# erikszasz/GaussianSplattingRegistration

Hardware: AMD Instinct MI355X
Metric: Gaussians/sec through HEM level + ICP iters/sec, 2x5M-splat pair (higher is better)
Workload: dtype f32 (HEM) / f64 (ICP)

## Files before the change

### gaussiansplattingregistration_amd/csrc/icp.hip

```cpp
#include "gsr_common.h"
#include "gsr_normals.h"
#include "gsr_solve.h"
#include "gsr_features.h"
#include "gsr_grid.h"
#include "gsr_oneshot.h"
#include "gsr_prims.h"

#include <float.h>
#include <math.h>
#include <stdlib.h>
#include <string.h>
#include <vector>

namespace gsr {
#ifndef GSR_ICP_MERGE_BS
#define GSR_ICP_MERGE_BS 1024
#define GSR_ICP_MERGE_IPT 4
#endif
using icp_merge_cfg = rocprim::merge_sort_config<512, GSR_ICP_MERGE_BS, GSR_ICP_MERGE_IPT, 128, 128, 4>;
using icp_sort_cfg = rocprim::radix_sort_config<rocprim::default_config, icp_merge_cfg,
                                                rocprim::radix_sort_onesweep_config<rocprim::kernel_config<1024, 16>, rocprim::kernel_config<1024, 16>, 11,
                                                                                    rocprim::block_radix_rank_algorithm::match>>;

#ifndef ICP_CELL_FLOOR_DIV
// ... 951 lines not shown
    const bool first = s_st.evals == 0;
    const bool stop = !first && fabs(s_st.fit - fit) < s_st.rel_fit && fabs(s_st.rmse - rmse) < s_st.rel_rmse;
    st->fit = fit; st->rmse = rmse;
    st->evals = s_st.evals + 1;
    if (stop || s_st.iters >= s_st.max_iter) { st->done = 1; return; }
    double update[16], T[16];
    estimate_update(s_st.ctr, s_st.kind, acc, update);
#pragma unroll
    for (int i = 0; i < 16; ++i) T[i] = s_st.T[i];
    mat4_mul(update, T, T);
#pragma unroll
    for (int i = 0; i < 16; ++i) st->T[i] = T[i];
    st->iters = s_st.iters + 1;
}
__global__ __launch_bounds__(ICP_STEP_THREADS) void k_icp_step(int nblocks, const double* __restrict__ partials, const double* __restrict__ reduced,
                                                   IcpState* __restrict__ st) {
    __shared__ double s_x[16][GSR_ICP_ACC_LEN];
    __shared__ IcpState s_st;
    static_assert(GSR_ICP_ACC_LEN == 32 && sizeof(IcpState) % 4 == 0, "k_icp_step layout");
    if (threadIdx.x < sizeof(IcpState) / 4) reinterpret_cast<int*>(&s_st)[threadIdx.x] = reinterpret_cast<const int*>(st)[threadIdx.x];
    icp_fold_partials<ICP_STEP_THREADS>(nblocks, partials, reduced, s_x);
    if (threadIdx.x != 0 || s_st.done) return;
    icp_step_solve(&s_x[0][0], s_st, st);
}

__global__ __launch_bounds__(1024) void k_icp_reduce(int nblocks, const double* __restrict__ partials, const IcpState* __restrict__ st,
                                                     double* __restrict__ out) {
    const int lane = threadIdx.x & 63, wv = threadIdx.x >> 6;
    const bool done = st->done != 0;
    for (int k = wv; k < GSR_ICP_ACC_LEN; k += 16) {
        double s = 0.0;
        if (!done)
            for (int b = lane; b < nblocks; b += 64) s += partials[(int64_t)b * GSR_ICP_ACC_LEN + k];
        for (int o = 32; o > 0; o >>= 1) s += __shfl_xor(s, o);
        if (lane == 0) out[k] = s;
    }
}

// ... 3 lines not shown

struct gsr_icp_ctx {
    int device = 0;
    hipStream_t stream = nullptr;
    IcpGrid grid;
    bool have_target = false, have_normals = false, have_source = false;
    int64_t nt = 0, ns = 0, ns_global = 0;
    double max_corr = 0;
    DevBuf src_raw, src_order, state, nn_j, Tc, Sc, stage_cov, Ti, Tg, Si;
    bool have_tcov = false, have_scov = false, have_tcol = false, have_scol = false;
    double lambda_geometric = 0.968;
    bool src_sorted = false;
    bool device_loop = true;
    bool block_search = true;
    bool xcd_ranges = true;
    gsr_comm* comm = nullptr;
    PinnedBlock host_rb;
    unsigned long long rb_seq = 0;
    int nn_kernel = -1;
    int nn_mode() const { return nn_kernel >= 0 ? (nn_kernel ? 2 : 0) : (ns >= 400000 ? 2 : 0); }
    double cell_target = 2.0;
    DevBuf hist;
    bool robust_box = false;
    bool robust_allowed = true;
    DevBuf bbox, keys, idx, skeys, order, cellStart, Tq, Tn, stage_xyz, stage_nrm, src, partials, acc_dev, rocprim_tmp, corr_idx, corr_d2;
    gsr_allreduce_fn allreduce = nullptr;
    void* allreduce_user = nullptr;
    gsr_allreduce_dev64_fn allreduce_dev = nullptr;
    void* allreduce_dev_user = nullptr;
    Event e0, e1, eb0, eb1;
    bool defer_sync = false;
    bool build_pending = false;
    float ms_build = 0, ms_iter = 0;
// ... 51 lines not shown
    const double* tn = p2p ? nullptr : (kind == GSR_ICP_GENERALIZED ? c->Tc.as<double>() : c->Tn.as<double>());
    const double* sc = kind == GSR_ICP_GENERALIZED ? c->Sc.as<double>() : nullptr;
    decltype(&k_icp_accumulate_dev<0, 0>) kernel = nullptr;
    switch (2 * kind + (blockf ? 1 : 0)) {
        case 0: kernel = k_icp_accumulate_dev<0, 0>; break;
        case 1: kernel = k_icp_accumulate_dev<0, 1>; break;
        case 2: kernel = k_icp_accumulate_dev<1, 0>; break;
        case 3: kernel = k_icp_accumulate_dev<1, 1>; break;
        case 4: kernel = k_icp_accumulate_dev<2, 0>; break;
        case 5: kernel = k_icp_accumulate_dev<2, 1>; break;
        case 6: kernel = k_icp_accumulate_dev<3, 0>; break;
        case 7: kernel = k_icp_accumulate_dev<3, 1>; break;
        case 8: kernel = k_icp_accumulate_dev<4, 0>; break;
        default: kernel = k_icp_accumulate_dev<4, 1>; break;
    }
    hipLaunchKernelGGL(kernel, dim3(8 * ((nb + 7) / 8)), dim3(256), 0, st, c->ns, c->src.as<float>(), c->state.as<IcpState>(), c->grid, c->cellStart.as<int>(), nnj,
                       c->Tq.as<float4>(), tn, sc, cargs, mc2, loss, k, c->partials.as<double>(), c->xcd_ranges ? nb : -nb);
}

int32_t run_accumulate(gsr_icp_ctx* c, const double* T, int kind, int loss, double k, double* acc, bool timed) {
    GSR_TRY(icp_check_kind(c, kind));
    hipStream_t st = c->stream;
    Xform X;
    for (int i = 0; i < 12; ++i) X.m[i] = T[i];
    const int nb = icp_blocks(c->ns, c->nblocks);
    GSR_TRY(c->partials.reserve((size_t)nb * GSR_ICP_ACC_LEN * 8));
    GSR_TRY(c->acc_dev.reserve(GSR_ICP_ACC_LEN * 8));
    GSR_HIP(hipMemsetAsync(c->partials.p, 0, (size_t)nb * GSR_ICP_ACC_LEN * 8, st));
    if (timed) GSR_HIP(hipEventRecord(c->e0, st));
    const double mc2 = c->max_corr * c->max_corr;
    const int* nnj = nullptr;
// ... 51 lines not shown
    unsigned* const host_rb = c->host_rb.as<unsigned>();
    if (!host_rb || bytes > 1024 || (bytes & 3)) {
        GSR_HIP(hipMemcpyAsync(out, dev, bytes, hipMemcpyDeviceToHost, st));
        GSR_HIP(hipStreamSynchronize(st));
        return GSR_OK;
    }
    const unsigned long long seq = ++c->rb_seq;
    unsigned long long* flag = reinterpret_cast<unsigned long long*>(host_rb + 256);
    hipLaunchKernelGGL(k_icp_publish, dim3(1), dim3(64), 0, st, (const unsigned*)dev, (int)(bytes >> 2), host_rb, flag, seq);
    GSR_HIP(hipGetLastError());
    GSR_TRY(wait_host_flag(st, flag, seq, true));
    memcpy(out, (const void*)host_rb, bytes);
    return GSR_OK;
}

int32_t gsr_icp_create(gsr_icp_ctx** out, int32_t device, void* stream) {
    if (!out) return fail(GSR_E_INVALID, "gsr_icp_create: out is NULL");
    *out = nullptr;
    int ndev = 0;
    if (hipGetDeviceCount(&ndev) != hipSuccess || ndev <= 0)
        return fail(GSR_E_NO_DEVICE, "gsr_icp_create: no HIP device visible (this backend has no CPU fallback)");
    if (device < 0 || device >= ndev) return fail(GSR_E_INVALID, "gsr_icp_create: device %d out of range", device);
    GSR_HIP(hipSetDevice(device));
    gsr_icp_ctx* c = new gsr_icp_ctx();
    c->device = device;
    c->stream = (hipStream_t)stream;
    if (c->e0.create() != hipSuccess || c->e1.create() != hipSuccess || c->eb0.create() != hipSuccess || c->eb1.create() != hipSuccess) {
        delete c; return fail(GSR_E_HIP, "hipEventCreate failed");
    }
    if (const char* e = getenv("GSR_ICP_DEVICE_LOOP")) c->device_loop = atoi(e) != 0;
    if (const char* e = getenv("GSR_ICP_BLOCK_SEARCH")) c->block_search = atoi(e) != 0;
    if (const char* e = getenv("GSR_ICP_XCD")) c->xcd_ranges = atoi(e) != 0;
    if (const char* e = getenv("GSR_ICP_ROBUST_BOX")) c->robust_allowed = atoi(e) != 0;
    if (const char* e = getenv("GSR_ICP_BLOCKS")) { int v = atoi(e); if (v >= 1 && v <= 65536) c->nblocks = v; }
    bool poll = true;
    if (const char* e = getenv("GSR_ICP_RB_POLL")) poll = atoi(e) != 0;
    if (!poll || c->host_rb.alloc(1024 + 64) != hipSuccess) (void)hipGetLastError();
    if (const char* e = getenv("GSR_ICP_NN_KERNEL")) c->nn_kernel = atoi(e);
    if (const char* e = getenv("GSR_ICP_CELL_TARGET")) { double v = atof(e); if (v > 0.01 && v < 1000) c->cell_target = v; }
    if (const char* e = getenv("GSR_ICP_MAX_CELLS")) { int v = atoi(e); if (v >= 1024) c->max_cells = v; }
    *out = c;
    return GSR_OK;
}

int32_t gsr_icp_destroy(gsr_icp_ctx* c) {
    delete c;
    return GSR_OK;
}

int32_t gsr_icp_set_target(gsr_icp_ctx* c, const float* xyz, const double* normals, int64_t n, double max_corr, int32_t on_device) {
    if (!c) return fail(GSR_E_INVALID, "gsr_icp_set_target: NULL context");
    if (!(max_corr > 0)) return fail(GSR_E_PRECONDITION, "max_correspondence_distance must be > 0 (got %g)", max_corr);
    if (n <= 0 || !xyz) return fail(GSR_E_PRECONDITION, "gsr_icp_set_target: empty target cloud");
    if (n >= ((int64_t)1 << 31) - 1) return fail(GSR_E_INVALID, "gsr_icp_set_target: n too large");
    GSR_HIP(hipSetDevice(c->device));
    hipStream_t st = c->stream;
    GSR_HIP(hipEventRecord(c->eb0, st));
    const float* dxyz = xyz;
    const double* dnrm = normals;
    if (!on_device) {
        GSR_TRY(c->stage_xyz.reserve((size_t)n * 12));
        GSR_HIP(hipMemcpyAsync(c->stage_xyz.p, xyz, (size_t)n * 12, hipMemcpyHostToDevice, st));
        dxyz = c->stage_xyz.as<float>();
        if (normals) {
            GSR_TRY(c->stage_nrm.reserve((size_t)n * 24));
            GSR_HIP(hipMemcpyAsync(c->stage_nrm.p, normals, (size_t)n * 24, hipMemcpyHostToDevice, st));
            dnrm = c->stage_nrm.as<double>();
        }
    }
    const int nbb = stride_grid(n);
    GSR_TRY(c->bbox.reserve(64 + (size_t)nbb * 24));
    hipLaunchKernelGGL(k_icp_bbox, dim3(nbb), dim3(256), 0, st, n, dxyz, c->bbox.as<float>() + 16);
    hipLaunchKernelGGL(k_icp_bbox_reduce, dim3(1), dim3(256), 0, st, nbb, c->bbox.as<float>() + 16, c->bbox.as<float>());
    GSR_TRY(c->hist.reserve(3 * ICP_HIST_BINS * 4));
    GSR_HIP(hipMemsetAsync(c->hist.p, 0, 3 * ICP_HIST_BINS * 4, st));
    hipLaunchKernelGGL(k_icp_hist, dim3(nbb > 512 ? 512 : nbb), dim3(256), 0, st, n, dxyz, c->bbox.as<float>(), c->hist.as<unsigned>());
    hipLaunchKernelGGL(k_icp_trim, dim3(1), dim3(64), 0, st, c->hist.as<unsigned>(), c->bbox.as<float>(), c->bbox.as<float>() + 6, c->bbox.as<float>() + 12);
    float hb[13];
    GSR_TRY(icp_fetch(c, c->bbox.p, hb, 13 * 4));
    const float raw_box[6] = {hb[0], hb[1], hb[2], hb[3], hb[4], hb[5]};
    c->robust_box = hb[12] != 0.0f && c->robust_allowed;
    if (c->robust_box) {
        GSR_HIP(hipMemsetAsync(c->hist.p, 0, 3 * ICP_HIST_BINS * 4, st));
        hipLaunchKernelGGL(k_icp_hist, dim3(nbb > 512 ? 512 : nbb), dim3(256), 0, st, n, dxyz, c->bbox.as<float>() + 6, c->hist.as<unsigned>());
        hipLaunchKernelGGL(k_icp_trim, dim3(1), dim3(64), 0, st, c->hist.as<unsigned>(), c->bbox.as<float>() + 6, c->bbox.as<float>(), c->bbox.as<float>() + 12);
        GSR_TRY(icp_fetch(c, c->bbox.p, hb, 6 * 4));
    }
    double mn[3], mx[3];
    for (int k = 0; k < 3; ++k) { mn[k] = hb[k]; mx[k] = hb[3 + k]; }
    IcpGrid g;
    if (!(mx[0] >= mn[0])) { mn[0] = mn[1] = mn[2] = 0; mx[0] = mx[1] = mx[2] = 0; }
    double cell;
    {
        const double ex = mx[0] - mn[0], ey = mx[1] - mn[1], ez = mx[2] - mn[2];
        const double emax = fmax(ex, fmax(ey, ez)), eps = emax * 1e-6 + 1e-30;
        cell = cbrt((ex + eps) * (ey + eps) * (ez + eps) * c->cell_target / (double)n);
        if (!(cell > 0)) cell = max_corr;
        if (cell < max_corr / ICP_CELL_FLOOR_DIV) cell = max_corr / ICP_CELL_FLOOR_DIV;
    }
    GSR_TRY(c->keys.reserve(n * 4)); GSR_TRY(c->idx.reserve(n * 4)); GSR_TRY(c->skeys.reserve(n * 4)); GSR_TRY(c->order.reserve(n * 4));
    for (;;) {
        double fx = floor((mx[0] - mn[0]) / cell) + 1, fy = floor((mx[1] - mn[1]) / cell) + 1, fz = floor((mx[2] - mn[2]) / cell) + 1;
        if (fx * fy * fz <= (double)c->max_cells) { g.gx = (int)fx; g.gy = (int)fy; g.gz = (int)fz; break; }
        cell *= 1.2599210498948732;
    }
    g.ox = mn[0]; g.oy = mn[1]; g.oz = mn[2];
    g.c = cell; g.inv_c = 1.0 / cell;
    g.cx = 0.5 * (mn[0] + mx[0]); g.cy = 0.5 * (mn[1] + mx[1]); g.cz = 0.5 * (mn[2] + mx[2]);
    g.ncells = g.gx * g.gy * g.gz;
    g.rings = (int)ceil(max_corr / cell);
    if (g.rings < 1) g.rings = 1;
    g.bx0 = raw_box[0]; g.by0 = raw_box[1]; g.bz0 = raw_box[2]; g.bx1 = raw_box[3]; g.by1 = raw_box[4]; g.bz1 = raw_box[5];
    if (!(raw_box[3] >= raw_box[0])) { g.bx0 = g.by0 = g.bz0 = -1.0 / 0.0; g.bx1 = g.by1 = g.bz1 = 1.0 / 0.0; }
    hipLaunchKernelGGL(k_icp_keys, dim3(stride_grid(n)), dim3(256), 0, st, n, dxyz, g, c->keys.as<unsigned>(), c->idx.as<unsigned>());
    int bits = 1;
    while (bits < 32 && ((int64_t)1 << bits) < g.ncells) ++bits;
    GSR_TRY(sort_pairs_by_key<icp_sort_cfg>(c->rocprim_tmp, st, c->keys.as<unsigned>(), c->skeys.as<unsigned>(), c->idx.as<unsigned>(),
                                            c->order.as<unsigned>(), (size_t)n, 0u, (unsigned)bits));
    GSR_TRY(c->cellStart.reserve(((size_t)g.ncells + 1) * 4));
    hipLaunchKernelGGL(k_icp_cell_starts, dim3(stride_grid(n)), dim3(256), 0, st, n, c->skeys.as<unsigned>(), (int64_t)g.ncells, c->cellStart.as<int>());
    c->grid = g;
    GSR_TRY(c->Tq.reserve((size_t)n * 16));
    if (normals) GSR_TRY(c->Tn.reserve((size_t)n * 24));
    hipLaunchKernelGGL(k_icp_gather_target, dim3(stride_grid(n)), dim3(256), 0, st, n, c->order.as<unsigned>(), dxyz, dnrm,
                       c->Tq.as<float4>(), normals ? c->Tn.as<double>() : (double*)nullptr);
    GSR_HIP(hipEventRecord(c->eb1, st));
    if (c->defer_sync) c->build_pending = true;
    else {
        GSR_HIP(hipStreamSynchronize(st));
        (void)hipEventElapsedTime(&c->ms_build, c->eb0, c->eb1);
        c->build_pending = false;
    }
    GSR_HIP(hipGetLastError());
    c->nt = n; c->max_corr = max_corr; c->have_target = true; c->have_normals = normals != nullptr;
    c->have_tcov = false; c->have_scov = false; c->have_tcol = false; c->have_scol = false;
    c->have_source = false;
    return GSR_OK;
}

int32_t gsr_icp_set_source(gsr_icp_ctx* c, const float* xyz, int64_t n, int32_t on_device) {
    if (!c) return fail(GSR_E_INVALID, "gsr_icp_set_source: NULL context");
    if (n < 0 || (n > 0 && !xyz)) return fail(GSR_E_PRECONDITION, "gsr_icp_set_source: empty source cloud");
    if (n >= ((int64_t)1 << 31) - 1) return fail(GSR_E_INVALID, "gsr_icp_set_source: n too large");
    GSR_HIP(hipSetDevice(c->device));
    hipStream_t st = c->stream;
    GSR_TRY(c->src.reserve((size_t)(n > 0 ? n : 1) * 12));
    c->src_sorted = false;
    if (n == 0) {
    } else if (c->have_target) {
        const float* raw = xyz;
        if (!on_device) {
            GSR_TRY(c->src_raw.reserve((size_t)n * 12));
            GSR_HIP(hipMemcpyAsync(c->src_raw.p, xyz, (size_t)n * 12, hipMemcpyHostToDevice, st));
            raw = c->src_raw.as<float>();
        }
        GSR_TRY(c->keys.reserve(n * 4)); GSR_TRY(c->idx.reserve(n * 4)); GSR_TRY(c->skeys.reserve(n * 4)); GSR_TRY(c->src_order.reserve(n * 4));
        hipLaunchKernelGGL(k_icp_keys, dim3(stride_grid(n)), dim3(256), 0, st, n, raw, c->grid, c->keys.as<unsigned>(), c->idx.as<unsigned>());
        int bits = 1;
// ... 116 lines not shown
    return GSR_OK;
}
int32_t gsr_icp_set_allreduce(gsr_icp_ctx* c, gsr_allreduce_fn fn, void* user, int64_t n_source_global) {
    if (!c) return fail(GSR_E_INVALID, "gsr_icp_set_allreduce: NULL context");
    c->allreduce = fn; c->allreduce_user = user;
    if (fn) { c->allreduce_dev = nullptr; c->allreduce_dev_user = nullptr; c->comm = nullptr; }
    c->ns_global = fn ? n_source_global : c->ns;
    return GSR_OK;
}

int32_t gsr_icp_accumulate(gsr_icp_ctx* c, const double* T, int32_t kind, int32_t loss, double k, double* acc) {
    GSR_TRY(icp_check_scaled(kind, loss, "gsr_icp_accumulate"));
    if (!c || !T || !acc) return fail(GSR_E_INVALID, "gsr_icp_accumulate: NULL argument");
    GSR_HIP(hipSetDevice(c->device));
    return run_accumulate(c, T, kind, loss, k, acc, false);
}

int32_t gsr_icp_register(gsr_icp_ctx* c, const double* init_T, int32_t kind, int32_t loss, double k, double rel_fitness,
                         double rel_rmse, int32_t max_iter, double* out_T, double* fitness, double* inlier_rmse, int32_t* iterations) {
    GSR_TRY(icp_check_scaled(kind, loss, "gsr_icp_register"));
    if (!c || !init_T || !out_T) return fail(GSR_E_INVALID, "gsr_icp_register: NULL argument");
    GSR_HIP(hipSetDevice(c->device));
    c->ms_iter = 0; c->n_iter_kernels = 0;
    const bool multi = c->allreduce_dev != nullptr || c->comm != nullptr;
    if (!c->allreduce && !multi && c->have_source && c->ns == 0)
        return fail(GSR_E_PRECONDITION, "gsr_icp_register: empty source cloud");
    if (!c->allreduce && (c->device_loop || multi)) {
        GSR_TRY(icp_check_kind(c, kind));
        hipStream_t st = c->stream;
        IcpState hs;
        memset(&hs, 0, sizeof(hs));
        memcpy(hs.T, init_T, sizeof(hs.T));
        hs.ctr[0] = c->grid.cx; hs.ctr[1] = c->grid.cy; hs.ctr[2] = c->grid.cz;
        hs.nsg = (double)(multi ? c->ns_global : c->ns); hs.rel_fit = rel_fitness; hs.rel_rmse = rel_rmse;
        hs.max_iter = max_iter < 0 ? 0 : max_iter; hs.kind = kind;
        GSR_TRY(c->state.reserve(sizeof(IcpState)));
        GSR_HIP(hipMemcpyAsync(c->state.p, &hs, sizeof(hs), hipMemcpyHostToDevice, st));
        const int nb = icp_blocks(c->ns, c->nblocks);
        GSR_TRY(c->partials.reserve((size_t)nb * GSR_ICP_ACC_LEN * 8));
        GSR_TRY(c->nn_j.reserve((size_t)(c->ns > 0 ? c->ns : 1) * 4));
        GSR_TRY(c->acc_dev.reserve(GSR_ICP_ACC_LEN * 8));
        GSR_HIP(hipMemsetAsync(c->partials.p, 0, (size_t)nb * GSR_ICP_ACC_LEN * 8, st));
        const double mc2 = c->max_corr * c->max_corr;
        const ColorArgs cargs = {c->Ti.as<double>(), c->Tg.as<double>(), c->Si.as<double>(), sqrt(c->lambda_geometric), sqrt(1.0 - c->lambda_geometric)};
        const int total_evals = hs.max_iter + 1;
        const bool blockf = c->block_search && c->grid.rings >= 2;
        int issued = 0;
        GSR_HIP(hipEventRecord(c->e0, st));
        while (issued < total_evals) {
            const int chunk = total_evals - issued < 8 ? total_evals - issued : 8;
            const int* nnj = c->nn_mode() ? c->nn_j.as<int>() : (const int*)nullptr;
            for (int i = 0; i < chunk; ++i) {
                if (c->nn_mode()) launch_icp_nn<true>(c, st, Xform(), c->state.as<IcpState>(), mc2, blockf);
                launch_accumulate_dev(c, st, kind, blockf, nb, nnj, cargs, mc2, loss, k);
                if (multi) {
                    hipLaunchKernelGGL(k_icp_reduce, dim3(1), dim3(1024), 0, st, nb, c->partials.as<double>(), c->state.as<IcpState>(), c->acc_dev.as<double>());
                    if (c->comm) {
                        GSR_TRY(gsr_comm_allreduce(c->comm, c->acc_dev.p, GSR_ICP_ACC_LEN, GSR_DT_F64, GSR_OP_SUM, (void*)st));
                    } else {
                        const int32_t rc = c->allreduce_dev(c->acc_dev.p, GSR_ICP_ACC_LEN, c->allreduce_dev_user);
                        if (rc != 0) return fail(GSR_E_INVALID, "icp: device all-reduce callback returned %d", rc);
                    }
                    hipLaunchKernelGGL(k_icp_step, dim3(1), dim3(ICP_STEP_THREADS), 0, st, nb, c->partials.as<double>(), c->acc_dev.as<double>(), c->state.as<IcpState>());
                } else {
                    hipLaunchKernelGGL(k_icp_step, dim3(1), dim3(ICP_STEP_THREADS), 0, st, nb, c->partials.as<double>(), (const double*)nullptr, c->state.as<IcpState>());
                }
            }
            issued += chunk;
            GSR_HIP(hipGetLastError());
            GSR_TRY(icp_fetch(c, c->state.p, &hs, sizeof(hs)));
            if (hs.done) break;
        }
        GSR_HIP(hipEventRecord(c->e1, st));
        GSR_HIP(hipStreamSynchronize(st));
        (void)hipEventElapsedTime(&c->ms_iter, c->e0, c->e1);
        c->n_iter_kernels = hs.evals;
        memcpy(out_T, hs.T, sizeof(hs.T));
        if (fitness) *fitness = hs.fit;
        if (inlier_rmse) *inlier_rmse = hs.rmse;
        if (iterations) *iterations = hs.iters;
        return GSR_OK;
    }
    double T[16], acc[GSR_ICP_ACC_LEN], update[16];
    memcpy(T, init_T, sizeof(T));
    GSR_TRY(run_accumulate(c, T, kind, loss, k, acc, true));
    const double nsg = (double)(c->ns_global > 0 ? c->ns_global : c->ns);
    double fit = acc[0] > 0 ? acc[0] / nsg : 0.0, rmse = acc[0] > 0 ? sqrt(acc[1] / acc[0]) : 0.0;
// ... 106 lines not shown
    if (!c) return fail(GSR_E_INVALID, "gsr_icp_register_clouds: NULL context");
    if (kind != GSR_ICP_POINT_TO_POINT && kind != GSR_ICP_POINT_TO_PLANE && kind != GSR_ICP_POINT_TO_POINT_SCALED)
        return fail(GSR_E_INVALID, "gsr_icp_register_clouds: point-to-point and point-to-plane only (covariances / colours: the step-by-step entry points)");
    if (kind == GSR_ICP_POINT_TO_PLANE && !tgt_normals) return fail(GSR_E_PRECONDITION, "TransformationEstimationPointToPlane requires target normals");
    c->comm = nullptr; c->allreduce = nullptr; c->allreduce_user = nullptr; c->allreduce_dev = nullptr; c->allreduce_dev_user = nullptr;
    c->defer_sync = c->device_loop;
    int32_t r = gsr_icp_set_target(c, tgt_xyz, kind == GSR_ICP_POINT_TO_PLANE ? tgt_normals : nullptr, nt, max_corr, on_device);
    if (r == GSR_OK) r = gsr_icp_set_source(c, src_xyz, ns, on_device);
    c->defer_sync = false;
    if (r == GSR_OK) { c->ns_global = ns; r = gsr_icp_register(c, init_T, kind, loss, k, rel_fitness, rel_rmse, max_iter, out_T, fitness, inlier_rmse, iterations); }
    if (r != GSR_OK) (void)hipStreamSynchronize(c->stream);
    icp_read_build_ms(c);
    return r;
}

int32_t gsr_icp_register_multiscale(gsr_icp_ctx* c, int32_t n_entries, const gsr_icp_entry* entries, int32_t on_device, const double* init_T, int32_t kind,
                                    int32_t loss, double k, double rel_fitness, double rel_rmse, gsr_icp_entry_result* results, double* out_T) {
    GSR_TRY(icp_check_scaled(kind, loss, "gsr_icp_register_multiscale"));
    if (!c || !init_T || !out_T || n_entries < 0 || (n_entries > 0 && (!entries || !results)))
        return fail(GSR_E_INVALID, "gsr_icp_register_multiscale: bad argument");
    double T[16];
    memcpy(T, init_T, sizeof(T));
    for (int e = 0; e < n_entries; ++e) {
        const gsr_icp_entry& E = entries[e];
        gsr_icp_entry_result& R = results[e];
        memset(&R, 0, sizeof(R));
        memcpy(R.init_T, T, sizeof(T));
        const int32_t r = gsr_icp_register_clouds(c, E.src_xyz, E.ns, E.tgt_xyz, E.tgt_normals, E.nt, on_device, E.max_corr, T, kind, loss, k, rel_fitness, rel_rmse,
                                                  E.max_iter, R.T, &R.fitness, &R.inlier_rmse, &R.iterations);
        if (r != GSR_OK) return r;
        R.ms_build = c->ms_build; R.ms_iters = c->ms_iter; R.evaluations = c->n_iter_kernels;
        memcpy(T, R.T, sizeof(T));
    }
    memcpy(out_T, T, sizeof(T));
    return GSR_OK;
// ... 159 lines not shown
```

Baseline: 577.0 million.

## Pipeline multiscale ICP levels on device with per-level state slots and host-word polling

Multiscale registration now computes every level's target bounding box in one batch, then enqueues each level's index build, source upload and device ICP loop back to back on the stream. Each level keeps its own state slot, and the next level's starting transform is chained on device from the previous slot, so the host does not synchronise between levels. A state-init kernel replaces the host-to-device state copy and the partials memset. The step kernel also writes a sequence-and-done word to host memory for cheaper polling. This removes host round-trips and stalls between levels, at the cost of more complex control flow and buffers sized to the largest level.

```diff
diff --git a/gaussiansplattingregistration_amd/csrc/icp.hip b/gaussiansplattingregistration_amd/csrc/icp.hip
--- a/gaussiansplattingregistration_amd/csrc/icp.hip
+++ b/gaussiansplattingregistration_amd/csrc/icp.hip
@@ -7,6 +7,7 @@
 #include "gsr_prims.h"
 
 #include <float.h>
+#include <stddef.h>
 #include <math.h>
 #include <stdlib.h>
 #include <string.h>
@@ -989,14 +990,15 @@
     st->iters = s_st.iters + 1;
 }
 __global__ __launch_bounds__(ICP_STEP_THREADS) void k_icp_step(int nblocks, const double* __restrict__ partials, const double* __restrict__ reduced,
-                                                   IcpState* __restrict__ st) {
+                                                   IcpState* __restrict__ st, unsigned long long* __restrict__ host_word, unsigned long long eval_seq) {
     __shared__ double s_x[16][GSR_ICP_ACC_LEN];
     __shared__ IcpState s_st;
     static_assert(GSR_ICP_ACC_LEN == 32 && sizeof(IcpState) % 4 == 0, "k_icp_step layout");
     if (threadIdx.x < sizeof(IcpState) / 4) reinterpret_cast<int*>(&s_st)[threadIdx.x] = reinterpret_cast<const int*>(st)[threadIdx.x];
     icp_fold_partials<ICP_STEP_THREADS>(nblocks, partials, reduced, s_x);
-    if (threadIdx.x != 0 || s_st.done) return;
-    icp_step_solve(&s_x[0][0], s_st, st);
+    if (threadIdx.x != 0) return;
+    if (!s_st.done) icp_step_solve(&s_x[0][0], s_st, st);
+    if (host_word) __hip_atomic_store(host_word, 2ull * eval_seq + (st->done != 0 ? 1ull : 0ull), __ATOMIC_RELAXED, __HIP_MEMORY_SCOPE_SYSTEM);
 }
 
 __global__ __launch_bounds__(1024) void k_icp_reduce(int nblocks, const double* __restrict__ partials, const IcpState* __restrict__ st,
@@ -1030,9 +1032,14 @@
     bool device_loop = true;
     bool block_search = true;
     bool xcd_ranges = true;
+    bool pipeline = true;
+    int state_slot = 0;
+    std::vector<Event> ms_ev;
+    IcpState* cur_state() const { return state.as<IcpState>() + state_slot; }
     gsr_comm* comm = nullptr;
     PinnedBlock host_rb;
     unsigned long long rb_seq = 0;
+    unsigned long long eval_seq = 0;
     int nn_kernel = -1;
     int nn_mode() const { return nn_kernel >= 0 ? (nn_kernel ? 2 : 0) : (ns >= 400000 ? 2 : 0); }
     double cell_target = 2.0;
@@ -1114,7 +1121,7 @@
         case 8: kernel = k_icp_accumulate_dev<4, 0>; break;
         default: kernel = k_icp_accumulate_dev<4, 1>; break;
     }
-    hipLaunchKernelGGL(kernel, dim3(8 * ((nb + 7) / 8)), dim3(256), 0, st, c->ns, c->src.as<float>(), c->state.as<IcpState>(), c->grid, c->cellStart.as<int>(), nnj,
+    hipLaunchKernelGGL(kernel, dim3(8 * ((nb + 7) / 8)), dim3(256), 0, st, c->ns, c->src.as<float>(), c->cur_state(), c->grid, c->cellStart.as<int>(), nnj,
                        c->Tq.as<float4>(), tn, sc, cargs, mc2, loss, k, c->partials.as<double>(), c->xcd_ranges ? nb : -nb);
 }
 
@@ -1196,6 +1203,16 @@
     return GSR_OK;
 }
 
+__global__ __launch_bounds__(256) void k_icp_state_init(IcpState init, const IcpState* __restrict__ prev, IcpState* __restrict__ st, double* __restrict__ partials,
+                                                        int64_t npartials) {
+    static_assert(offsetof(IcpState, T) == 0 && sizeof(IcpState) / 4 <= 256, "k_icp_state_init layout");
+    for (int64_t i = (int64_t)blockIdx.x * blockDim.x + threadIdx.x; i < npartials; i += (int64_t)gridDim.x * blockDim.x) partials[i] = 0.0;
+    if (blockIdx.x == 0 && threadIdx.x < sizeof(IcpState) / 4) {
+        const unsigned w = threadIdx.x;
+        const unsigned v = (prev && w < 32u) ? reinterpret_cast<const unsigned*>(prev)[w] : reinterpret_cast<const unsigned*>(&init)[w];
+        reinterpret_cast<unsigned*>(st)[w] = v;
+    }
+}
 int32_t gsr_icp_create(gsr_icp_ctx** out, int32_t device, void* stream) {
     if (!out) return fail(GSR_E_INVALID, "gsr_icp_create: out is NULL");
     *out = nullptr;
@@ -1213,6 +1230,7 @@
     if (const char* e = getenv("GSR_ICP_DEVICE_LOOP")) c->device_loop = atoi(e) != 0;
     if (const char* e = getenv("GSR_ICP_BLOCK_SEARCH")) c->block_search = atoi(e) != 0;
     if (const char* e = getenv("GSR_ICP_XCD")) c->xcd_ranges = atoi(e) != 0;
+    if (const char* e = getenv("GSR_ICP_PIPELINE")) c->pipeline = atoi(e) != 0;
     if (const char* e = getenv("GSR_ICP_ROBUST_BOX")) c->robust_allowed = atoi(e) != 0;
     if (const char* e = getenv("GSR_ICP_BLOCKS")) { int v = atoi(e); if (v >= 1 && v <= 65536) c->nblocks = v; }
     bool poll = true;
@@ -1230,11 +1248,96 @@
     return GSR_OK;
 }
 
-int32_t gsr_icp_set_target(gsr_icp_ctx* c, const float* xyz, const double* normals, int64_t n, double max_corr, int32_t on_device) {
-    if (!c) return fail(GSR_E_INVALID, "gsr_icp_set_target: NULL context");
+static int32_t icp_reserve_boxes(gsr_icp_ctx* c, int nslots, int64_t n_max) {
+    GSR_TRY(c->bbox.reserve(64 * (size_t)nslots + (size_t)stride_grid(n_max) * 24));
+    return c->hist.reserve(3 * ICP_HIST_BINS * 4);
+}
+static int32_t icp_enqueue_box(gsr_icp_ctx* c, int nslots, int slot, int64_t n, const float* dxyz) {
+    hipStream_t st = c->stream;
+    const int nbb = stride_grid(n);
+    float* part = c->bbox.as<float>() + 16 * nslots;
+    float* hdr = c->bbox.as<float>() + 16 * slot;
+    hipLaunchKernelGGL(k_icp_bbox, dim3(nbb), dim3(256), 0, st, n, dxyz, part);
+    hipLaunchKernelGGL(k_icp_bbox_reduce, dim3(1), dim3(256), 0, st, nbb, part, hdr);
+    GSR_HIP(hipMemsetAsync(c->hist.p, 0, 3 * ICP_HIST_BINS * 4, st));
+    hipLaunchKernelGGL(k_icp_hist, dim3(nbb > 512 ? 512 : nbb), dim3(256), 0, st, n, dxyz, hdr, c->hist.as<unsigned>());
+    hipLaunchKernelGGL(k_icp_trim, dim3(1), dim3(64), 0, st, c->hist.as<unsigned>(), hdr, hdr + 6, hdr + 12);
+    return GSR_OK;
+}
+static int32_t icp_enqueue_box_refine(gsr_icp_ctx* c, int slot, int64_t n, const float* dxyz) {
+    hipStream_t st = c->stream;
+    const int nbb = stride_grid(n);
+    float* hdr = c->bbox.as<float>() + 16 * slot;
+    GSR_HIP(hipMemsetAsync(c->hist.p, 0, 3 * ICP_HIST_BINS * 4, st));
+    hipLaunchKernelGGL(k_icp_hist, dim3(nbb > 512 ? 512 : nbb), dim3(256), 0, st, n, dxyz, hdr + 6, c->hist.as<unsigned>());
+    hipLaunchKernelGGL(k_icp_trim, dim3(1), dim3(64), 0, st, c->hist.as<unsigned>(), hdr + 6, hdr, hdr + 12);
+    return GSR_OK;
+}
+static IcpGrid icp_make_grid(const gsr_icp_ctx* c, const float* box, const float* raw_box, int64_t n, double max_corr) {
+    double mn[3], mx[3];
+    for (int k = 0; k < 3; ++k) { mn[k] = box[k]; mx[k] = box[3 + k]; }
+    IcpGrid g;
+    if (!(mx[0] >= mn[0])) { mn[0] = mn[1] = mn[2] = 0; mx[0] = mx[1] = mx[2] = 0; }
+    double cell;
+    {
+        const double ex = mx[0] - mn[0], ey = mx[1] - mn[1], ez = mx[2] - mn[2];
+        const double emax = fmax(ex, fmax(ey, ez)), eps = emax * 1e-6 + 1e-30;
+        cell = cbrt((ex + eps) * (ey + eps) * (ez + eps) * c->cell_target / (double)n);
+        if (!(cell > 0)) cell = max_corr;
+        if (cell < max_corr / ICP_CELL_FLOOR_DIV) cell = max_corr / ICP_CELL_FLOOR_DIV;
+    }
+    for (;;) {
+        double fx = floor((mx[0] - mn[0]) / cell) + 1, fy = floor((mx[1] - mn[1]) / cell) + 1, fz = floor((mx[2] - mn[2]) / cell) + 1;
+        if (fx * fy * fz <= (double)c->max_cells) { g.gx = (int)fx; g.gy = (int)fy; g.gz = (int)fz; break; }
+        cell *= 1.2599210498948732;
+    }
+    g.ox = mn[0]; g.oy = mn[1]; g.oz = mn[2];
+    g.c = cell; g.inv_c = 1.0 / cell;
+    g.cx = 0.5 * (mn[0] + mx[0]); g.cy = 0.5 * (mn[1] + mx[1]); g.cz = 0.5 * (mn[2] + mx[2]);
+    g.ncells = g.gx * g.gy * g.gz;
+    g.rings = (int)ceil(max_corr / cell);
+    if (g.rings < 1) g.rings = 1;
+    g.bx0 = raw_box[0]; g.by0 = raw_box[1]; g.bz0 = raw_box[2]; g.bx1 = raw_box[3]; g.by1 = raw_box[4]; g.bz1 = raw_box[5];
+    if (!(raw_box[3] >= raw_box[0])) { g.bx0 = g.by0 = g.bz0 = -1.0 / 0.0; g.bx1 = g.by1 = g.bz1 = 1.0 / 0.0; }
+    return g;
+}
+static int32_t icp_enqueue_index(gsr_icp_ctx* c, int64_t n, const float* dxyz, const double* dnrm, const IcpGrid& g) {
+    hipStream_t st = c->stream;
+    GSR_TRY(c->keys.reserve(n * 4)); GSR_TRY(c->idx.reserve(n * 4)); GSR_TRY(c->skeys.reserve(n * 4)); GSR_TRY(c->order.reserve(n * 4));
+    hipLaunchKernelGGL(k_icp_keys, dim3(stride_grid(n)), dim3(256), 0, st, n, dxyz, g, c->keys.as<unsigned>(), c->idx.as<unsigned>());
+    int bits = 1;
+    while (bits < 32 && ((int64_t)1 << bits) < g.ncells) ++bits;
+    GSR_TRY(sort_pairs_by_key<icp_sort_cfg>(c->rocprim_tmp, st, c->keys.as<unsigned>(), c->skeys.as<unsigned>(), c->idx.as<unsigned>(),
+                                            c->order.as<unsigned>(), (size_t)n, 0u, (unsigned)bits));
+    GSR_TRY(c->cellStart.reserve(((size_t)g.ncells + 1) * 4));
+    hipLaunchKernelGGL(k_icp_cell_starts, dim3(stride_grid(n)), dim3(256), 0, st, n, c->skeys.as<unsigned>(), (int64_t)g.ncells, c->cellStart.as<int>());
+    c->grid = g;
+    GSR_TRY(c->Tq.reserve((size_t)n * 16));
+    if (dnrm) GSR_TRY(c->Tn.reserve((size_t)n * 24));
+    hipLaunchKernelGGL(k_icp_gather_target, dim3(stride_grid(n)), dim3(256), 0, st, n, c->order.as<unsigned>(), dxyz, dnrm,
+                       c->Tq.as<float4>(), dnrm ? c->Tn.as<double>() : (double*)nullptr);
+    return GSR_OK;
+}
+static void icp_target_is(gsr_icp_ctx* c, int64_t n, double max_corr, bool normals, bool robust_box) {
+    c->nt = n; c->max_corr = max_corr; c->have_target = true; c->have_normals = normals; c->robust_box = robust_box;
+    c->have_tcov = false; c->have_scov = false; c->have_tcol = false; c->have_scol = false;
+    c->have_source = false;
+}
+static int32_t icp_check_target_args(const float* xyz, int64_t n, double max_corr) {
     if (!(max_corr > 0)) return fail(GSR_E_PRECONDITION, "max_correspondence_distance must be > 0 (got %g)", max_corr);
     if (n <= 0 || !xyz) return fail(GSR_E_PRECONDITION, "gsr_icp_set_target: empty target cloud");
     if (n >= ((int64_t)1 << 31) - 1) return fail(GSR_E_INVALID, "gsr_icp_set_target: n too large");
+    return GSR_OK;
+}
+static int32_t icp_check_source_args(const float* xyz, int64_t n) {
+    if (n < 0 || (n > 0 && !xyz)) return fail(GSR_E_PRECONDITION, "gsr_icp_set_source: empty source cloud");
+    if (n >= ((int64_t)1 << 31) - 1) return fail(GSR_E_INVALID, "gsr_icp_set_source: n too large");
+    return GSR_OK;
+}
+
+int32_t gsr_icp_set_target(gsr_icp_ctx* c, const float* xyz, const double* normals, int64_t n, double max_corr, int32_t on_device) {
+    if (!c) return fail(GSR_E_INVALID, "gsr_icp_set_target: NULL context");
+    GSR_TRY(icp_check_target_args(xyz, n, max_corr));
     GSR_HIP(hipSetDevice(c->device));
     hipStream_t st = c->stream;
     GSR_HIP(hipEventRecord(c->eb0, st));
@@ -1250,62 +1353,17 @@
             dnrm = c->stage_nrm.as<double>();
         }
     }
-    const int nbb = stride_grid(n);
-    GSR_TRY(c->bbox.reserve(64 + (size_t)nbb * 24));
-    hipLaunchKernelGGL(k_icp_bbox, dim3(nbb), dim3(256), 0, st, n, dxyz, c->bbox.as<float>() + 16);
-    hipLaunchKernelGGL(k_icp_bbox_reduce, dim3(1), dim3(256), 0, st, nbb, c->bbox.as<float>() + 16, c->bbox.as<float>());
-    GSR_TRY(c->hist.reserve(3 * ICP_HIST_BINS * 4));
-    GSR_HIP(hipMemsetAsync(c->hist.p, 0, 3 * ICP_HIST_BINS * 4, st));
-    hipLaunchKernelGGL(k_icp_hist, dim3(nbb > 512 ? 512 : nbb), dim3(256), 0, st, n, dxyz, c->bbox.as<float>(), c->hist.as<unsigned>());
-    hipLaunchKernelGGL(k_icp_trim, dim3(1), dim3(64), 0, st, c->hist.as<unsigned>(), c->bbox.as<float>(), c->bbox.as<float>() + 6, c->bbox.as<float>() + 12);
+    GSR_TRY(icp_reserve_boxes(c, 1, n));
+    GSR_TRY(icp_enqueue_box(c, 1, 0, n, dxyz));
     float hb[13];
     GSR_TRY(icp_fetch(c, c->bbox.p, hb, 13 * 4));
     const float raw_box[6] = {hb[0], hb[1], hb[2], hb[3], hb[4], hb[5]};
-    c->robust_box = hb[12] != 0.0f && c->robust_allowed;
-    if (c->robust_box) {
-        GSR_HIP(hipMemsetAsync(c->hist.p, 0, 3 * ICP_HIST_BINS * 4, st));
-        hipLaunchKernelGGL(k_icp_hist, dim3(nbb > 512 ? 512 : nbb), dim3(256), 0, st, n, dxyz, c->bbox.as<float>() + 6, c->hist.as<unsigned>());
-        hipLaunchKernelGGL(k_icp_trim, dim3(1), dim3(64), 0, st, c->hist.as<unsigned>(), c->bbox.as<float>() + 6, c->bbox.as<float>(), c->bbox.as<float>() + 12);
+    const bool robust = hb[12] != 0.0f && c->robust_allowed;
+    if (robust) {
+        GSR_TRY(icp_enqueue_box_refine(c, 0, n, dxyz));
         GSR_TRY(icp_fetch(c, c->bbox.p, hb, 6 * 4));
     }
-    double mn[3], mx[3];
-    for (int k = 0; k < 3; ++k) { mn[k] = hb[k]; mx[k] = hb[3 + k]; }
-    IcpGrid g;
-    if (!(mx[0] >= mn[0])) { mn[0] = mn[1] = mn[2] = 0; mx[0] = mx[1] = mx[2] = 0; }
-    double cell;
-    {
-        const double ex = mx[0] - mn[0], ey = mx[1] - mn[1], ez = mx[2] - mn[2];
-        const double emax = fmax(ex, fmax(ey, ez)), eps = emax * 1e-6 + 1e-30;
-        cell = cbrt((ex + eps) * (ey + eps) * (ez + eps) * c->cell_target / (double)n);
-        if (!(cell > 0)) cell = max_corr;
-        if (cell < max_corr / ICP_CELL_FLOOR_DIV) cell = max_corr / ICP_CELL_FLOOR_DIV;
-    }
-    GSR_TRY(c->keys.reserve(n * 4)); GSR_TRY(c->idx.reserve(n * 4)); GSR_TRY(c->skeys.reserve(n * 4)); GSR_TRY(c->order.reserve(n * 4));
-    for (;;) {
-        double fx = floor((mx[0] - mn[0]) / cell) + 1, fy = floor((mx[1] - mn[1]) / cell) + 1, fz = floor((mx[2] - mn[2]) / cell) + 1;
-        if (fx * fy * fz <= (double)c->max_cells) { g.gx = (int)fx; g.gy = (int)fy; g.gz = (int)fz; break; }
-        cell *= 1.2599210498948732;
-    }
-    g.ox = mn[0]; g.oy = mn[1]; g.oz = mn[2];
-    g.c = cell; g.inv_c = 1.0 / cell;
-    g.cx = 0.5 * (mn[0] + mx[0]); g.cy = 0.5 * (mn[1] + mx[1]); g.cz = 0.5 * (mn[2] + mx[2]);
-    g.ncells = g.gx * g.gy * g.gz;
-    g.rings = (int)ceil(max_corr / cell);
-    if (g.rings < 1) g.rings = 1;
-    g.bx0 = raw_box[0]; g.by0 = raw_box[1]; g.bz0 = raw_box[2]; g.bx1 = raw_box[3]; g.by1 = raw_box[4]; g.bz1 = raw_box[5];
-    if (!(raw_box[3] >= raw_box[0])) { g.bx0 = g.by0 = g.bz0 = -1.0 / 0.0; g.bx1 = g.by1 = g.bz1 = 1.0 / 0.0; }
-    hipLaunchKernelGGL(k_icp_keys, dim3(stride_grid(n)), dim3(256), 0, st, n, dxyz, g, c->keys.as<unsigned>(), c->idx.as<unsigned>());
-    int bits = 1;
-    while (bits < 32 && ((int64_t)1 << bits) < g.ncells) ++bits;
-    GSR_TRY(sort_pairs_by_key<icp_sort_cfg>(c->rocprim_tmp, st, c->keys.as<unsigned>(), c->skeys.as<unsigned>(), c->idx.as<unsigned>(),
-                                            c->order.as<unsigned>(), (size_t)n, 0u, (unsigned)bits));
-    GSR_TRY(c->cellStart.reserve(((size_t)g.ncells + 1) * 4));
-    hipLaunchKernelGGL(k_icp_cell_starts, dim3(stride_grid(n)), dim3(256), 0, st, n, c->skeys.as<unsigned>(), (int64_t)g.ncells, c->cellStart.as<int>());
-    c->grid = g;
-    GSR_TRY(c->Tq.reserve((size_t)n * 16));
-    if (normals) GSR_TRY(c->Tn.reserve((size_t)n * 24));
-    hipLaunchKernelGGL(k_icp_gather_target, dim3(stride_grid(n)), dim3(256), 0, st, n, c->order.as<unsigned>(), dxyz, dnrm,
-                       c->Tq.as<float4>(), normals ? c->Tn.as<double>() : (double*)nullptr);
+    GSR_TRY(icp_enqueue_index(c, n, dxyz, dnrm, icp_make_grid(c, hb, raw_box, n, max_corr)));
     GSR_HIP(hipEventRecord(c->eb1, st));
     if (c->defer_sync) c->build_pending = true;
     else {
@@ -1314,16 +1372,13 @@
         c->build_pending = false;
     }
     GSR_HIP(hipGetLastError());
-    c->nt = n; c->max_corr = max_corr; c->have_target = true; c->have_normals = normals != nullptr;
-    c->have_tcov = false; c->have_scov = false; c->have_tcol = false; c->have_scol = false;
-    c->have_source = false;
+    icp_target_is(c, n, max_corr, normals != nullptr, robust);
     return GSR_OK;
 }
 
 int32_t gsr_icp_set_source(gsr_icp_ctx* c, const float* xyz, int64_t n, int32_t on_device) {
     if (!c) return fail(GSR_E_INVALID, "gsr_icp_set_source: NULL context");
-    if (n < 0 || (n > 0 && !xyz)) return fail(GSR_E_PRECONDITION, "gsr_icp_set_source: empty source cloud");
-    if (n >= ((int64_t)1 << 31) - 1) return fail(GSR_E_INVALID, "gsr_icp_set_source: n too large");
+    GSR_TRY(icp_check_source_args(xyz, n));
     GSR_HIP(hipSetDevice(c->device));
     hipStream_t st = c->stream;
     GSR_TRY(c->src.reserve((size_t)(n > 0 ? n : 1) * 12));
@@ -1470,6 +1525,104 @@
     if (!c || !T || !acc) return fail(GSR_E_INVALID, "gsr_icp_accumulate: NULL argument");
     GSR_HIP(hipSetDevice(c->device));
     return run_accumulate(c, T, kind, loss, k, acc, false);
+}
+
+static int icp_ahead(int64_t ns) { return ns >= 1000000 ? 1 : 4; }
+
+static int32_t icp_begin_loop(gsr_icp_ctx* c, const IcpState& hs, const IcpState* prev) {
+    hipStream_t st = c->stream;
+    GSR_TRY(c->state.reserve(sizeof(IcpState) * (size_t)(c->state_slot + 1)));
+    const int nb = icp_blocks(c->ns, c->nblocks);
+    GSR_TRY(c->partials.reserve((size_t)nb * GSR_ICP_ACC_LEN * 8));
+    GSR_TRY(c->nn_j.reserve((size_t)(c->ns > 0 ? c->ns : 1) * 4));
+    GSR_TRY(c->acc_dev.reserve(GSR_ICP_ACC_LEN * 8));
+    if (c->pipeline) {
+        const int64_t np = (int64_t)nb * GSR_ICP_ACC_LEN;
+        hipLaunchKernelGGL(k_icp_state_init, dim3(stride_grid(np)), dim3(256), 0, st, hs, prev, c->cur_state(), c->partials.as<double>(), np);
+        return GSR_OK;
+    }
+    GSR_HIP(hipMemcpyAsync(c->cur_state(), &hs, sizeof(hs), hipMemcpyHostToDevice, st));
+    GSR_HIP(hipMemsetAsync(c->partials.p, 0, (size_t)nb * GSR_ICP_ACC_LEN * 8, st));
+    return GSR_OK;
+}
+
+static volatile unsigned long long* icp_progress_word(const gsr_icp_ctx* c) {
+    return c->host_rb.as<unsigned>() ? reinterpret_cast<volatile unsigned long long*>(c->host_rb.as<unsigned>() + 256) + 1 : nullptr;
+}
+static int32_t icp_wait_eval(gsr_icp_ctx* c, unsigned long long seq, bool* done) {
+    volatile unsigned long long* word = icp_progress_word(c);
+    unsigned long long v = 0;
+    const auto t0 = std::chrono::steady_clock::now();
+    for (unsigned spins = 1; ((v = __atomic_load_n(word, __ATOMIC_ACQUIRE)) >> 1) < seq; ++spins) {
+        if ((spins & 0x3ffu) == 0u && std::chrono::steady_clock::now() - t0 > std::chrono::milliseconds(200)) {
+            GSR_HIP(hipStreamSynchronize(c->stream));
+            v = __atomic_load_n(word, __ATOMIC_ACQUIRE);
+            if ((v >> 1) < seq) return fail(GSR_E_HIP, "icp: evaluation %llu never reported (the stream is idle at %llu)", seq, v >> 1);
+            break;
+        }
+        cpu_relax(spins);
+    }
+    *done = (v & 1ull) != 0;
+    return GSR_OK;
+}
+
+static int32_t icp_run_loop(gsr_icp_ctx* c, int kind, int loss, double k, int total_evals, bool multi, bool final_wait, IcpState* hs) {
+    hipStream_t st = c->stream;
+    const int nb = icp_blocks(c->ns, c->nblocks);
+    const double mc2 = c->max_corr * c->max_corr;
+    const ColorArgs cargs = {c->Ti.as<double>(), c->Tg.as<double>(), c->Si.as<double>(), sqrt(c->lambda_geometric), sqrt(1.0 - c->lambda_geometric)};
+    const bool blockf = c->block_search && c->grid.rings >= 2;
+    volatile unsigned long long* const word = icp_progress_word(c);
+    const bool ahead = c->pipeline && !multi && word != nullptr;
+    IcpState* const state = c->cur_state();
+    const int* const nnj = c->nn_mode() ? c->nn_j.as<int>() : (const int*)nullptr;
+    if (ahead) {
+        const int behind = icp_ahead(c->ns);
+        const unsigned long long first = c->eval_seq + 1;
+        for (int issued = 0; issued < total_evals;) {
+            if (c->nn_mode()) launch_icp_nn<true>(c, st, Xform(), state, mc2, blockf);
+            launch_accumulate_dev(c, st, kind, blockf, nb, nnj, cargs, mc2, loss, k);
+            hipLaunchKernelGGL(k_icp_step, dim3(1), dim3(ICP_STEP_THREADS), 0, st, nb, c->partials.as<double>(), (const double*)nullptr, state,
+                               const_cast<unsigned long long*>(word), ++c->eval_seq);
+            ++issued;
+            GSR_HIP(hipGetLastError());
+            bool done = false;
+            if (issued > behind) GSR_TRY(icp_wait_eval(c, first + (unsigned long long)(issued - behind) - 1, &done));
+            else {
+                const unsigned long long v = __atomic_load_n(word, __ATOMIC_ACQUIRE);
+                done = (v >> 1) >= first && (v & 1ull) != 0;
+            }
+            if (done) break;
+        }
+        return final_wait ? icp_fetch(c, state, hs, sizeof(*hs)) : GSR_OK;
+    }
+    int issued = 0;
+    while (issued < total_evals) {
+        const int chunk = total_evals - issued < 8 ? total_evals - issued : 8;
+        for (int i = 0; i < chunk; ++i) {
+            if (c->nn_mode()) launch_icp_nn<true>(c, st, Xform(), state, mc2, blockf);
+            launch_accumulate_dev(c, st, kind, blockf, nb, nnj, cargs, mc2, loss, k);
+            if (multi) {
+                hipLaunchKernelGGL(k_icp_reduce, dim3(1), dim3(1024), 0, st, nb, c->partials.as<double>(), state, c->acc_dev.as<double>());
+                if (c->comm) {
+                    GSR_TRY(gsr_comm_allreduce(c->comm, c->acc_dev.p, GSR_ICP_ACC_LEN, GSR_DT_F64, GSR_OP_SUM, (void*)st));
+                } else {
+                    const int32_t rc = c->allreduce_dev(c->acc_dev.p, GSR_ICP_ACC_LEN, c->allreduce_dev_user);
+                    if (rc != 0) return fail(GSR_E_INVALID, "icp: device all-reduce callback returned %d", rc);
+                }
+                hipLaunchKernelGGL(k_icp_step, dim3(1), dim3(ICP_STEP_THREADS), 0, st, nb, c->partials.as<double>(), c->acc_dev.as<double>(), state,
+                                   (unsigned long long*)nullptr, 0ull);
+            } else {
+                hipLaunchKernelGGL(k_icp_step, dim3(1), dim3(ICP_STEP_THREADS), 0, st, nb, c->partials.as<double>(), (const double*)nullptr, state,
+                                   (unsigned long long*)nullptr, 0ull);
+            }
+        }
+        issued += chunk;
+        GSR_HIP(hipGetLastError());
+        GSR_TRY(icp_fetch(c, state, hs, sizeof(*hs)));
+        if (hs->done) break;
+    }
+    return GSR_OK;
 }
 
 int32_t gsr_icp_register(gsr_icp_ctx* c, const double* init_T, int32_t kind, int32_t loss, double k, double rel_fitness,
@@ -1490,43 +1643,10 @@
         hs.ctr[0] = c->grid.cx; hs.ctr[1] = c->grid.cy; hs.ctr[2] = c->grid.cz;
         hs.nsg = (double)(multi ? c->ns_global : c->ns); hs.rel_fit = rel_fitness; hs.rel_rmse = rel_rmse;
         hs.max_iter = max_iter < 0 ? 0 : max_iter; hs.kind = kind;
-        GSR_TRY(c->state.reserve(sizeof(IcpState)));
-        GSR_HIP(hipMemcpyAsync(c->state.p, &hs, sizeof(hs), hipMemcpyHostToDevice, st));
-        const int nb = icp_blocks(c->ns, c->nblocks);
-        GSR_TRY(c->partials.reserve((size_t)nb * GSR_ICP_ACC_LEN * 8));
-        GSR_TRY(c->nn_j.reserve((size_t)(c->ns > 0 ? c->ns : 1) * 4));
-        GSR_TRY(c->acc_dev.reserve(GSR_ICP_ACC_LEN * 8));
-        GSR_HIP(hipMemsetAsync(c->partials.p, 0, (size_t)nb * GSR_ICP_ACC_LEN * 8, st));
-        const double mc2 = c->max_corr * c->max_corr;
-        const ColorArgs cargs = {c->Ti.as<double>(), c->Tg.as<double>(), c->Si.as<double>(), sqrt(c->lambda_geometric), sqrt(1.0 - c->lambda_geometric)};
-        const int total_evals = hs.max_iter + 1;
-        const bool blockf = c->block_search && c->grid.rings >= 2;
-        int issued = 0;
+        c->state_slot = 0;
+        GSR_TRY(icp_begin_loop(c, hs, nullptr));
         GSR_HIP(hipEventRecord(c->e0, st));
-        while (issued < total_evals) {
-            const int chunk = total_evals - issued < 8 ? total_evals - issued : 8;
-            const int* nnj = c->nn_mode() ? c->nn_j.as<int>() : (const int*)nullptr;
-            for (int i = 0; i < chunk; ++i) {
-                if (c->nn_mode()) launch_icp_nn<true>(c, st, Xform(), c->state.as<IcpState>(), mc2, blockf);
-                launch_accumulate_dev(c, st, kind, blockf, nb, nnj, cargs, mc2, loss, k);
-                if (multi) {
-                    hipLaunchKernelGGL(k_icp_reduce, dim3(1), dim3(1024), 0, st, nb, c->partials.as<double>(), c->state.as<IcpState>(), c->acc_dev.as<double>());
-                    if (c->comm) {
-                        GSR_TRY(gsr_comm_allreduce(c->comm, c->acc_dev.p, GSR_ICP_ACC_LEN, GSR_DT_F64, GSR_OP_SUM, (void*)st));
-                    } else {
-                        const int32_t rc = c->allreduce_dev(c->acc_dev.p, GSR_ICP_ACC_LEN, c->allreduce_dev_user);
-                        if (rc != 0) return fail(GSR_E_INVALID, "icp: device all-reduce callback returned %d", rc);
-                    }
-                    hipLaunchKernelGGL(k_icp_step, dim3(1), dim3(ICP_STEP_THREADS), 0, st, nb, c->partials.as<double>(), c->acc_dev.as<double>(), c->state.as<IcpState>());
-                } else {
-                    hipLaunchKernelGGL(k_icp_step, dim3(1), dim3(ICP_STEP_THREADS), 0, st, nb, c->partials.as<double>(), (const double*)nullptr, c->state.as<IcpState>());
-                }
-            }
-            issued += chunk;
-            GSR_HIP(hipGetLastError());
-            GSR_TRY(icp_fetch(c, c->state.p, &hs, sizeof(hs)));
-            if (hs.done) break;
-        }
+        GSR_TRY(icp_run_loop(c, kind, loss, k, hs.max_iter + 1, multi, true, &hs));
         GSR_HIP(hipEventRecord(c->e1, st));
         GSR_HIP(hipStreamSynchronize(st));
         (void)hipEventElapsedTime(&c->ms_iter, c->e0, c->e1);
@@ -1663,11 +1783,115 @@
     return r;
 }
 
+static int32_t icp_check_entry(const gsr_icp_entry& E, int kind) {
+    if (kind != GSR_ICP_POINT_TO_POINT && kind != GSR_ICP_POINT_TO_PLANE && kind != GSR_ICP_POINT_TO_POINT_SCALED)
+        return fail(GSR_E_INVALID, "gsr_icp_register_clouds: point-to-point and point-to-plane only (covariances / colours: the step-by-step entry points)");
+    if (kind == GSR_ICP_POINT_TO_PLANE && !E.tgt_normals) return fail(GSR_E_PRECONDITION, "TransformationEstimationPointToPlane requires target normals");
+    GSR_TRY(icp_check_target_args(E.tgt_xyz, E.nt, E.max_corr));
+    GSR_TRY(icp_check_source_args(E.src_xyz, E.ns));
+    if (E.ns == 0) return fail(GSR_E_PRECONDITION, "gsr_icp_register: empty source cloud");
+    return GSR_OK;
+}
+
+static int32_t icp_multiscale_pipelined(gsr_icp_ctx* c, int32_t n_entries, const gsr_icp_entry* entries, const double* init_T, int32_t kind, int32_t loss,
+                                        double k, double rel_fitness, double rel_rmse, gsr_icp_entry_result* results, double* out_T) {
+    hipStream_t st = c->stream;
+    while (c->ms_ev.size() < (size_t)3 * n_entries + 1) {
+        Event ev;
+        if (ev.create() != hipSuccess) return fail(GSR_E_HIP, "hipEventCreate failed");
+        c->ms_ev.push_back(std::move(ev));
+    }
+    const bool normals = kind == GSR_ICP_POINT_TO_PLANE;
+    int64_t nt_max = 0, ns_max = 0;
+    for (int e = 0; e < n_entries; ++e) {
+        if (entries[e].nt > nt_max) nt_max = entries[e].nt;
+        if (entries[e].ns > ns_max) ns_max = entries[e].ns;
+    }
+    GSR_TRY(icp_reserve_boxes(c, n_entries, nt_max));
+    for (int e = 0; e < n_entries; ++e) GSR_TRY(icp_enqueue_box(c, n_entries, e, entries[e].nt, entries[e].tgt_xyz));
+    std::vector<float> raw((size_t)16 * n_entries), box;
+    GSR_TRY(icp_fetch(c, c->bbox.p, raw.data(), (size_t)64 * n_entries));
+    std::vector<char> robust(n_entries, 0);
+    bool any_robust = false;
+    for (int e = 0; e < n_entries; ++e)
+        if (raw[16 * e + 12] != 0.0f && c->robust_allowed) {
+            robust[e] = 1; any_robust = true;
+            GSR_TRY(icp_enqueue_box_refine(c, e, entries[e].nt, entries[e].tgt_xyz));
+        }
+    box = raw;
+    if (any_robust) GSR_TRY(icp_fetch(c, c->bbox.p, box.data(), (size_t)64 * n_entries));
+    std::vector<IcpGrid> grids(n_entries);
+    int64_t ncells_max = 0;
+    for (int e = 0; e < n_entries; ++e) {
+        grids[e] = icp_make_grid(c, (robust[e] ? box.data() : raw.data()) + 16 * e, raw.data() + 16 * e, entries[e].nt, entries[e].max_corr);
+        if (grids[e].ncells > ncells_max) ncells_max = grids[e].ncells;
+    }
+    {
+        const size_t nk = (size_t)(nt_max > ns_max ? nt_max : ns_max) * 4;
+        GSR_TRY(c->keys.reserve(nk)); GSR_TRY(c->idx.reserve(nk)); GSR_TRY(c->skeys.reserve(nk)); GSR_TRY(c->order.reserve((size_t)nt_max * 4));
+        GSR_TRY(c->src_order.reserve((size_t)ns_max * 4)); GSR_TRY(c->src.reserve((size_t)ns_max * 12)); GSR_TRY(c->nn_j.reserve((size_t)ns_max * 4));
+        GSR_TRY(c->cellStart.reserve(((size_t)ncells_max + 1) * 4)); GSR_TRY(c->Tq.reserve((size_t)nt_max * 16));
+        if (normals) GSR_TRY(c->Tn.reserve((size_t)nt_max * 24));
+        GSR_TRY(c->partials.reserve((size_t)icp_blocks(ns_max, c->nblocks) * GSR_ICP_ACC_LEN * 8));
+        GSR_TRY(c->state.reserve(sizeof(IcpState) * (size_t)n_entries));
+    }
+    for (int e = 0; e < n_entries; ++e) {
+        const gsr_icp_entry& E = entries[e];
+        if (e == 0) GSR_HIP(hipEventRecord(c->ms_ev[0], st));
+        GSR_TRY(icp_enqueue_index(c, E.nt, E.tgt_xyz, normals ? E.tgt_normals : nullptr, grids[e]));
+        GSR_HIP(hipEventRecord(c->ms_ev[3 * e + 1], st));
+        icp_target_is(c, E.nt, E.max_corr, normals, robust[e] != 0);
+        c->defer_sync = true;
+        const int32_t r = gsr_icp_set_source(c, E.src_xyz, E.ns, 1);
+        c->defer_sync = false;
+        GSR_TRY(r);
+        c->ns_global = E.ns;
+        GSR_TRY(icp_check_kind(c, kind));
+        IcpState hs;
+        memset(&hs, 0, sizeof(hs));
+        memcpy(hs.T, init_T, sizeof(hs.T));
+        hs.ctr[0] = c->grid.cx; hs.ctr[1] = c->grid.cy; hs.ctr[2] = c->grid.cz;
+        hs.nsg = (double)c->ns; hs.rel_fit = rel_fitness; hs.rel_rmse = rel_rmse;
+        hs.max_iter = E.max_iter < 0 ? 0 : E.max_iter; hs.kind = kind;
+        c->state_slot = e;
+        GSR_TRY(icp_begin_loop(c, hs, e > 0 ? c->state.as<IcpState>() + (e - 1) : (const IcpState*)nullptr));
+        GSR_HIP(hipEventRecord(c->ms_ev[3 * e + 2], st));
+        GSR_TRY(icp_run_loop(c, kind, loss, k, hs.max_iter + 1, false, false, &hs));
+        GSR_HIP(hipEventRecord(c->ms_ev[3 * e + 3], st));
+    }
+    GSR_HIP(hipGetLastError());
+    std::vector<IcpState> fin(n_entries);
+    GSR_HIP(hipMemcpyAsync(fin.data(), c->state.p, sizeof(IcpState) * (size_t)n_entries, hipMemcpyDeviceToHost, st));
+    GSR_HIP(hipStreamSynchronize(st));
+    for (int e = 0; e < n_entries; ++e) {
+        gsr_icp_entry_result& R = results[e];
+        memset(&R, 0, sizeof(R));
+        memcpy(R.init_T, e > 0 ? fin[e - 1].T : init_T, sizeof(R.init_T));
+        memcpy(R.T, fin[e].T, sizeof(R.T));
+        R.fitness = fin[e].fit; R.inlier_rmse = fin[e].rmse; R.iterations = fin[e].iters; R.evaluations = fin[e].evals;
+        (void)hipEventElapsedTime(&R.ms_build, c->ms_ev[3 * e], c->ms_ev[3 * e + 1]);
+        (void)hipEventElapsedTime(&R.ms_iters, c->ms_ev[3 * e + 2], c->ms_ev[3 * e + 3]);
+    }
+    const gsr_icp_entry_result& L = results[n_entries - 1];
+    c->ms_build = L.ms_build; c->ms_iter = L.ms_iters; c->n_iter_kernels = L.evaluations; c->build_pending = false;
+    c->state_slot = 0;
+    memcpy(out_T, L.T, sizeof(L.T));
+    return GSR_OK;
+}
+
 int32_t gsr_icp_register_multiscale(gsr_icp_ctx* c, int32_t n_entries, const gsr_icp_entry* entries, int32_t on_device, const double* init_T, int32_t kind,
                                     int32_t loss, double k, double rel_fitness, double rel_rmse, gsr_icp_entry_result* results, double* out_T) {
     GSR_TRY(icp_check_scaled(kind, loss, "gsr_icp_register_multiscale"));
     if (!c || !init_T || !out_T || n_entries < 0 || (n_entries > 0 && (!entries || !results)))
         return fail(GSR_E_INVALID, "gsr_icp_register_multiscale: bad argument");
+    for (int e = 0; e < n_entries; ++e) GSR_TRY(icp_check_entry(entries[e], kind));
+    if (n_entries > 0 && on_device && c->pipeline && c->device_loop) {
+        GSR_HIP(hipSetDevice(c->device));
+        c->comm = nullptr; c->allreduce = nullptr; c->allreduce_user = nullptr; c->allreduce_dev = nullptr; c->allreduce_dev_user = nullptr;
+        const int32_t r = icp_multiscale_pipelined(c, n_entries, entries, init_T, kind, loss, k, rel_fitness, rel_rmse, results, out_T);
+        if (r != GSR_OK) { (void)hipStreamSynchronize(c->stream); c->state_slot = 0; c->defer_sync = false; }
+        return r;
+    }
     double T[16];
     memcpy(T, init_T, sizeof(T));
     for (int e = 0; e < n_entries; ++e) {
```

Result: no change. 578.1 million (median of 2 runs) (+0.2%).
